# bnbowman/pbccs

Measured on AMD Instinct MI355X. Metric: CCS ZMWs/sec (and GCUPS) at 1/2/4/8 MI355X vs host-CPU ccs, higher is better.
Workload: dtype f64

## Files before the change

pbccs_amd/csrc/arrow_kernels.hip:

```cpp
#include "arrow_device.hpp"
#include "arrow_kernels.hpp"
#include "arrow_score_device.hpp"
#include "coop_chain.hpp"

#include <climits>

namespace pbccs {

__device__ __forceinline__ LaneBand scratch_band(const FillScratch& F, int g, int l, int which)
{
    const long long gm = 2LL * g + which;
    LaneBand m;
    m.range = F.range + gm * F.capCols * 64 + l;
    m.off = F.off + gm * F.capCols * 64 + l;
    m.ls = F.ls + gm * F.capCols * 64 + l;
    m.val = F.val + gm * F.capSlots * 64 + l;
    m.cap = F.capSlots;
    return m;
}

__global__ void __launch_bounds__(64) k_fill(DevBatch B, FillScratch F, const int* __restrict__ reads, int n)
{
    const int t = blockIdx.x * blockDim.x + threadIdx.x;
    if (t >= n) return;
    const int g = t >> 6, l = t & 63;
    const long long tStart = F.trace ? (long long)wall_clock64() : 0;
    const int r = reads[t];
    const int z = B.rZmw[r];
    const int I = B.rLen[r];
    const TplView tv = window_view(B, r);
    const int J = tv.Length();
    if (I < 1 || J < 1 || J + 2 > F.capCols) {
        B.rStatus[r] = (I < 1 || J < 1) ? kFillBadInput : kFillOverflow;
        return;
    }
    const char* rd = B.seqPool + B.rSeqOff[r];
    const Params P = params_for(B, z);
    const LaneBand a = scratch_band(F, g, l, 0);
// ... 140 lines not shown
                if (ok[q] && c < ncol[q]) {
                    const long long bits = __double_as_longlong(tile[ln][q]);
                    (which ? B.bRange : B.aRange)[cb[q] + c] = make_int2((int)(bits & 0xffffffff), (int)(bits >> 32));
                }
            }
            __syncthreads();
            for (int q = w; q < 64; q += 4) {
                const int c = c0 + q;
                tile[q][ln] = __longlong_as_double((c < maxC) ? (long long)F.off[gm + (long long)c * 64 + ln] : 0LL);
            }
            __syncthreads();
            for (int q = w; q < 64; q += 4) {
                const int c = c0 + ln;
                if (ok[q] && c < ncol[q]) (which ? B.bOff : B.aOff)[cb[q] + c] = (int)__double_as_longlong(tile[ln][q]);
            }
            __syncthreads();
        }
        const double* pre = F.pre + (long long)g * (F.capCols + 1) * 64;
        for (int q = w; q < 64; q += 4) {
            const int c = c0 + q;
            tile[q][ln] = (c < maxC + 1) ? pre[(long long)c * 64 + ln] : 0.0;
        }
        __syncthreads();
        for (int q = w; q < 64; q += 4) {
            const int c = c0 + ln;
            if (ok[q] && c < ncol[q] + 1) B.aPre[cb[q] + c] = tile[ln][q];
        }
        __syncthreads();
    }
}

constexpr int kSuffixTile = 2048;

__device__ __forceinline__ double add8(double s, const double* __restrict__ t)
{
    double v[8];
#pragma unroll
    for (int i = 0; i < 8; ++i) v[i] = t[i];
#pragma unroll
    for (int i = 0; i < 8; ++i) s = s + v[i];
    return s;
}

__device__ __forceinline__ void k_suffix_body(DevBatch B, const int* __restrict__ reads, int n, int withPrefix)
{
    __shared__ double tile[kSuffixTile];
    const int r = reads[blockIdx.x];
    if (B.rStatus[r] != kFillOk && B.rStatus[r] != kFillMismatch) return;
    const long long cb = B.rColBase[r];
    const int J = window_view(B, r).Length();
    const double* ls = B.bLs + cb;
    double* suf = B.bSuf + cb;
    const int ncol = J + 1;
    const int lane = threadIdx.x & 63;
    const int wbase = threadIdx.x & ~63;
    for (int k0 = 0; k0 <= ncol; k0 += blockDim.x) {
        const int kb = k0 + wbase;
        const int k = kb + lane;
        double s = 0.0;
        for (int c0 = k0; c0 < ncol; c0 += kSuffixTile) {
            __syncthreads();
            for (int q = threadIdx.x; q < kSuffixTile && c0 + q < ncol; q += blockDim.x) tile[q] = ls[c0 + q];
            __syncthreads();
            const int hi = min(ncol - c0, kSuffixTile);
            int q = max(kb - c0, 0);
            const int headEnd = min(hi, kb + 64 - c0);
            for (; q < headEnd; ++q) {
                const double v = tile[q];
                if (c0 + q >= k) s = s + v;
            }
            for (; q + 8 <= hi; q += 8) s = add8(s, tile + q);
            for (; q < hi; ++q) s = s + tile[q];
        }
        if (k <= ncol) suf[k] = s;
    }
    if (!withPrefix) return;
    if (threadIdx.x != 0) return;
    const double* als = B.aLs + cb;
    double* pre = B.aPre + cb;
    double run = 0.0;
    pre[0] = 0.0;
    int k = 0;
    for (; k + 8 <= ncol; k += 8) {
        double v[8];
#pragma unroll
        for (int q = 0; q < 8; ++q) v[q] = als[k + q];
#pragma unroll
        for (int q = 0; q < 8; ++q) {
            run = run + v[q];
            pre[k + q + 1] = run;
        }
    }
    for (; k < ncol; ++k) {
        run = run + als[k];
        pre[k + 1] = run;
    }
}
__global__ void __launch_bounds__(256) k_suffix(DevBatch B, const int* __restrict__ reads, int n, int withPrefix)
{
    const long long wt0 = wave_t0(B.stats);
    k_suffix_body(B, reads, n, withPrefix);
    wave_ticks(B.stats, kWaveSuffix, wt0);
}

__global__ void __launch_bounds__(256) k_enumerate(DevBatch B, const int* __restrict__ zmws,
                                                   const long long* __restrict__ mutBase,
                                                   const long long* __restrict__ posBase, int* __restrict__ codes,
                                                   int* __restrict__ posOff)
{
    __shared__ int waveSums[4];
    __shared__ int carry;
    const int z = zmws[blockIdx.x];
    const char* T = B.tplPool + B.zFwdOff[z];
    const int L = B.zLen[z];
    int* out = codes + mutBase[blockIdx.x];
    int* po = posOff + posBase[blockIdx.x];
    if (threadIdx.x == 0) carry = 0;
    __syncthreads();
    const int lane = threadIdx.x & 63, wid = threadIdx.x >> 6;
    for (int p0 = 0; p0 < L; p0 += 256) {
        const int p = p0 + threadIdx.x;
        int cnt = 0;
        char cur = 0, prev = '-';
        if (p < L) {
            cur = T[p];
            prev = p > 0 ? T[p - 1] : '-';
            cnt = (p == 0) ? 8 : 6 + (cur != prev ? 1 : 0);
        }
        int incl = cnt;
        for (int d = 1; d < 64; d <<= 1) {
            const int y = __shfl_up(incl, d, 64);
            if (lane >= d) incl += y;
        }
        if (lane == 63) waveSums[wid] = incl;
// ... 943 lines not shown
    int tagSub = -1, tagIns = -1;
    for (int m = po[p]; m < po[p + 1]; ++m) {
        const double s = sc[m];
        const int c = code[m];
        const int type = mut_type(c);
        const double e = s < 0.0 ? exp(s) : 0.0;
        part[0] += type == kIns ? e : 0.0;
        part[1] += type == kDel ? e : 0.0;
        part[2] += type == kSub ? e : 0.0;
        if (type == kSub && (tagSub < 0 || s > bestSub)) { bestSub = s; tagSub = mut_base(c); }
        if (type == kIns && (tagIns < 0 || s > bestIns)) { bestIns = s; tagIns = mut_base(c); }
    }
    const long long o = qvBase[k] + p;
    qv[o] = sum_to_qv(sum);
    R.ins[o] = sum_to_qv(part[0]);
    R.del[o] = sum_to_qv(part[1]);
    R.sub[o] = sum_to_qv(part[2]);
    R.subTag[o] = tagSub < 0 ? 'N' : base_char(tagSub);
    R.insTag[o] = tagIns < 0 ? 'N' : base_char(tagIns);
}

void launch_fill(const DevBatch& B, const FillScratch& F, const int* reads, int n, hipStream_t s)
{
    if (n <= 0) return;
    hipLaunchKernelGGL(k_fill, dim3((n + 63) / 64), dim3(64), 0, s, B, F, reads, n);
}

void launch_compact(const DevBatch& B, const FillScratch& F, const int* reads, int n, hipStream_t s)
{
    if (n <= 0) return;
    hipLaunchKernelGGL(k_compact, dim3((n + 63) / 64), dim3(256), 0, s, B, F, reads, n);
}

void launch_suffix(const DevBatch& B, const int* reads, int n, hipStream_t s, bool withPrefix)
{
    if (n <= 0) return;
    hipLaunchKernelGGL(k_suffix, dim3(n), dim3(256), 0, s, B, reads, n, withPrefix ? 1 : 0);
}

void launch_enumerate(const DevBatch& B, const int* zmws, int n, const long long* mutBase, const long long* posBase,
                      int* codes, int* posOff, hipStream_t s)
{
    if (n <= 0) return;
    hipLaunchKernelGGL(k_enumerate, dim3(n), dim3(256), 0, s, B, zmws, mutBase, posBase, codes, posOff);
}

void launch_score(const DevBatch& B, const ScoreWork& W, long long nWaves, const ScoreScratch& scratch, hipStream_t s,
                  const CkptWork* ck)
{
    if (nWaves <= 0) return;
    const long long blocks = (nWaves + kScoreWaves - 1) / kScoreWaves;
    hipLaunchKernelGGL(k_score, dim3((unsigned)blocks), dim3(64 * kScoreWaves), 0, s, B, W, scratch);
    if (ck && ck->nTasks > 0 && ck->nSlots > 0)
        hipLaunchKernelGGL(k_score_ckpt, dim3((unsigned)ck->nSlots), dim3(64), 0, s, B, W, *ck);
    if (W.edgeCap > 0)
        hipLaunchKernelGGL(k_score_edge, dim3((W.edgeCap + 63) / 64), dim3(64), 0, s, B, W, scratch);
}

void launch_reduce(const DevBatch& B, const ScoreWork& W, long long nMut, double fastThr, double* score,
                   unsigned char* fav, hipStream_t s)
{
    if (nMut <= 0) return;
    hipLaunchKernelGGL(k_reduce, dim3((unsigned)((nMut + 255) / 256)), dim3(256), 0, s, B, W, fastThr, score, fav);
}

void launch_alive(const DevBatch& B, const ScoreWork& W, long long nMut, double fastThr, int readHi,
                  unsigned char* alive, hipStream_t s)
{
    if (nMut <= 0) return;
    hipLaunchKernelGGL(k_alive, dim3((unsigned)((nMut + 255) / 256)), dim3(256), 0, s, B, W, fastThr, readHi, alive);
// ... 35 lines not shown
```

pbccs_amd/csrc/arrow_kernels.hpp:

```cpp
#pragma once

#include <hip/hip_runtime.h>

#include "arrow_device.hpp"

namespace pbccs {

struct ScoreWork {
    int nWork = 0;
    const int* zmw = nullptr;
    const int* nMut = nullptr;
    const long long* mutBase = nullptr;
    const long long* deltaBase = nullptr;
    const long long* waveStart = nullptr;
    const long long* mutStart = nullptr;
    const long long* posStart = nullptr;
    const int* codes = nullptr;
    double* delta = nullptr;
    int* edgeList = nullptr;
    int* edgeCount = nullptr;
    int edgeCap = 0;
    int readLo = 0;
    int readHi = 1 << 30;
    const long long* sel = nullptr;
// ... 59 lines not shown
    int* maxH = nullptr;
    int hcap = 0;
    int readWords = 0;
    int tplWords = 0;
    size_t groupBytes = 0;
    bool prio = false;
    bool chainExit = true;
    bool scan = false;
    double devScale = 1.0;
    int rows = 1;
    double thrMargin = 0x1p-50;
    int regrowSlackDiv = 16;
    unsigned long long* valBump = nullptr;
    long long valLimit = 0;
    long long* rValA = nullptr;
    long long* rValB = nullptr;
    long long* rValCap = nullptr;
    double* colScratch = nullptr;
    int gRows = 0;
    long long* trace = nullptr;
    unsigned long long* work = nullptr;
};
enum FillWork : int {
    kFillWorkCells = 0, kFillWorkTallAbort, kFillWorkRegrow, kFillWorkOverflow, kFillWorkSteps, kFillWorkIssues,
    kFillWorkReads, kFillWorkPasses, kFillWorkSlots
};
size_t coop_group_bytes(int hcap, int readWords, int tplWords);
constexpr int kNarrowGroupLanes = 16;
constexpr int kTallRowsPerLane = 2;
void launch_fill_coop(int G, const DevBatch& B, const CoopFill& F, const int* reads, int n, hipStream_t s);

void launch_fill(const DevBatch& B, const FillScratch& F, const int* reads, int n, hipStream_t s);
void launch_compact(const DevBatch& B, const FillScratch& F, const int* reads, int n, hipStream_t s);
void launch_suffix(const DevBatch& B, const int* reads, int n, hipStream_t s, bool withPrefix = false);
void launch_enumerate(const DevBatch& B, const int* zmws, int n, const long long* mutBase, const long long* posBase,
                      int* codes, int* posOff, hipStream_t s);
void launch_score(const DevBatch& B, const ScoreWork& W, long long nWaves, const ScoreScratch& scratch, hipStream_t s,
                  const CkptWork* ck = nullptr);
void launch_alive(const DevBatch& B, const ScoreWork& W, long long nMut, double fastThr, int readHi,
                  unsigned char* alive, hipStream_t s);
void launch_sel_ranges(const ScoreWork& W, const long long* sel, const long long* count, long long* selBase,
                       int* nSel, hipStream_t s);
void launch_score_wide(const DevBatch& B, const WideTask* tasks, int n, double* delta, hipStream_t s);
void launch_score_wide_refill(const DevBatch& B, const WideTask* tasks, int n, double* delta,
                              const ScoreScratch& scratch, int rowsCap, hipStream_t s);
void launch_reduce(const DevBatch& B, const ScoreWork& W, long long nMut, double fastThr, double* score,
                   unsigned char* fav, hipStream_t s);
void launch_best_subset(int nWork, const long long* selBase, const int* nSel, const int* code, const double* score,
                        int sep, int ldsCap, int* rank, hipStream_t s);
void launch_qv(const DevBatch& B, const ScoreWork& W, long long nPos, const long long* posBase, const int* posOff,
               const double* score, const long long* qvBase, int* qv, hipStream_t s);
struct RichQvOut {
    int* sub = nullptr;
    int* ins = nullptr;
    int* del = nullptr;
    char* subTag = nullptr;
    char* insTag = nullptr;
};
void launch_qv_rich(const DevBatch& B, const ScoreWork& W, long long nPos, const long long* posBase, const int* posOff,
                    const double* score, const long long* qvBase, int* qv, const RichQvOut& R, hipStream_t s);

}
```

pbccs_amd/csrc/engine.hip:

```cpp
#include "engine.hpp"
#include "diploid_kernels.hpp"
#include "refine_repeats.hpp"
#include "strand_kernels.hpp"

#include <hipcub/hipcub.hpp>

#include <algorithm>
#include <mutex>
#include <climits>
#include <cmath>
#include <cstdio>
#include <cstdlib>
#include <cstring>
#include <numeric>
#include <set>
#include <stdexcept>
#include <chrono>
#include <unordered_set>

namespace pbccs {

#define PBCCS_HIP(x)                                                         \
    do {                                                                     \
        hipError_t e_ = (x);                                                 \
        if (e_ != hipSuccess) throw DeviceError(hipGetErrorString(e_));      \
    } while (0)

const char* const kKernelNames[kKernelKinds] = {"k_fill",       "k_suffix",      "k_enumerate", "k_score",
                                                 "k_reduce",     "k_qv",          "k_best_subset", "k_compact",
                                                 "k_fill_tall",  "k_qfill_grp",   "k_qfill_coop", "k_qfill",
                                                 "k_qscore_mid", "k_qscore_multi", "k_score_wide", "k_qv_rich",
                                                 "k_strand_sums", "k_strand_sites"};

namespace {

constexpr int kFillBandHeight = 28;
constexpr double kFillScratchBudget = 24.0 * (1ull << 30);
constexpr int kCoopNarrowRows = 64;
constexpr int kCoopTallRows = 1024;
constexpr size_t kCoopLdsBytes = 60 * 1024;
constexpr int kHybridRows = 1536;
constexpr size_t kHeadroomMargin = 24ull << 30;
constexpr long long kTallFirstDiv = 25;
constexpr int kCkptDefaultK = 8;
constexpr int kCkptDefaultMinLen = 4000;
constexpr int kCkptSlotsMax = 2048;
constexpr long long kCkptSlotBytes = 1ll << 30;
int env_int(const char* name, int dflt)
{
    const char* e = std::getenv(name);
    return e ? std::atoi(e) : dflt;
}
constexpr long long kPhasedMinTasks = 1 << 21;
constexpr size_t kInitialScratch = 1 << 20;
constexpr int kMaxCopySegs = 8;

template <class T>
void upload(DevVec<T>& d, const std::vector<T>& h, hipStream_t s)
{
    d.reserve(std::max<size_t>(h.size(), 1), false);
    if (!h.empty()) PBCCS_HIP(hipMemcpyAsync(d.ptr, h.data(), h.size() * sizeof(T), hipMemcpyHostToDevice, s));
}

void d2h(void* dst, const void* src, size_t bytes, hipStream_t s)
{
    static const bool drain = env_int("PBCCS_D2H_DRAIN", 1) != 0;
    if (!bytes) return;
    if (drain) PBCCS_HIP(hipStreamSynchronize(s));
    PBCCS_HIP(hipMemcpyAsync(dst, src, bytes, hipMemcpyDeviceToHost, s));
}

template <class T>
void download(std::vector<T>& h, const DevVec<T>& d, size_t n, hipStream_t s)
{
    h.resize(n);
    d2h(h.data(), d.ptr, n * sizeof(T), s);
}

struct CopySeg {
    const unsigned int* src;
    unsigned int* dst;
    unsigned long long words;
};
struct CopySegs {
// ... 835 lines not shown
    b.prThird = kMismatchProbability / 3.0;
    b.sdn = zmws_.empty() ? std::exp(12.5) : std::exp(zmws_[0].opt.scoreDiff);
    b.stats = profiling_ ? dStats_.ptr : nullptr;
    return b;
}

void ArrowBatch::FillReads(const std::vector<int>& readsIn)
{
    const StreamScope bound(stream_);
    constexpr int kPaths = 4;
    for (int r : readsIn) EnsureCapacity(r);
    auto promote = [&](int r, int p) {
        HRead& h = reads_[r];
        int q = p + 1;
        if (q == 2 && (long long)h.seq.size() + 1 > 4LL * kCoopTallRows) q = 3;
        h.fillPath = q;
        if (q >= 2 && q < kPaths) {
            const long long I = (long long)h.seq.size(), J = h.te - h.ts;
            const bool ck = ckptAll_ > 0 || (ckptK_ > 0 && J >= ckptMinLen_);
            const long long K = ck ? std::max(ckptAll_, ckptK_) : 1;
            const long long want = (I + 1) * (J + 1) / kTallFirstDiv / K + (ck ? 2 * (kCkptTail + 1) * (I + 1) : 0) + 64;
            if (want > h.valCap) {
                h.valCap = want;
                h.valA = valTop_;
                h.valB = valTop_ + h.valCap;
                valTop_ += 2 * h.valCap;
                descDirty_ = true;
            }
        }
        return q;
    };
    Relayout(readsIn);
    const int firstPath = std::min(std::max(env_int("PBCCS_FILL_FIRST_PATH", 1), 1), 3);
    std::vector<int> todo[kPaths], serial, done;
    for (int r : readsIn) {
        if (reads_[r].fillPath < firstPath) reads_[r].fillPath = firstPath;
        const int p = reads_[r].fillPath;
        if (p >= kPaths) serial.push_back(r);
        else todo[p].push_back(r);
    }
    auto words = [&](int r) {
        return (int)(reads_[r].seq.size() + 7) / 8 + (reads_[r].te - reads_[r].ts + 8) / 8;
    };
    constexpr int tallG = 64;
    const int tallRows = env_int("PBCCS_TALL_ROWS", kTallRowsPerLane) == 1 ? 1 : 2;
    const long long chunk = (long long)tallG * tallRows;
    const long long tallGroupLds = (long long)kCoopLdsBytes;
    auto full_rows = [&](int maxI) { return ((long long)maxI + chunk) / chunk * chunk; };
    constexpr int narrowG = kNarrowGroupLanes;
    constexpr int narrowRows = 1;
    auto rows_for = [&](int p, int maxI, int w) -> int {
        if (p == 0) return 0;
        if (p == 1)
            return (64 / narrowG) * coop_group_bytes(kCoopNarrowRows, w, 0) <= kCoopLdsBytes
                       ? kCoopNarrowRows : 0;
        const long long room = (tallGroupLds - (long long)coop_group_bytes(0, w, 0)) / 16 / 64 * 64;
        const long long full = full_rows(maxI);
        if (p == 2) {
            const long long want = std::min<long long>(kCoopTallRows, full);
            return room >= want ? (int)want : 0;
        }
        const long long hybLds = (long long)env_int("PBCCS_HYBRID_LDS_KB", (int)(kCoopLdsBytes >> 10)) << 10;
        const long long hybRows = env_int("PBCCS_HYBRID_ROWS", kHybridRows);
        const long long hroom = (std::min<long long>(hybLds, 160 << 10) - (long long)coop_group_bytes(0, w, 0)) / 16 / 64 * 64;
        const long long want = std::min(std::min(full, hroom), hybRows);
        return want >= 64 ? (int)want : 0;
// ... 65 lines not shown
        std::vector<int> list;
        for (auto& v : todo) list.insert(list.end(), v.begin(), v.end());
        upload(dList_, list, stream_);
        const DevBatch B = View();
        size_t off = 0;
        const bool forked = !todo[2].empty() || !todo[3].empty();
        const auto tLaunch = std::chrono::steady_clock::now();
        const bool grow = ws_->val.allowVmm;
        long long headroom = 0;
        if (grow) {
            long long want = 1ll << 24;
            for (int p = 2; p < kPaths; ++p)
                for (int r : todo[p]) {
                    const long long I = (long long)reads_[r].seq.size(), J = reads_[r].te - reads_[r].ts;
                    const long long K = std::max(1, reads_[r].ckpt);
                    want += 2 * std::max<long long>(0, (I + 1) * (J + 1) / 7 / K - reads_[r].valCap);
                }
            size_t freeB = 0, totalB = 0;
            PBCCS_HIP(hipMemGetInfo(&freeB, &totalB));
            static const long long margin = (long long)env_int("PBCCS_HEADROOM_MARGIN_GB", (int)(kHeadroomMargin >> 30)) << 30;
            const long long spare = std::max<long long>(0, (long long)freeB - margin);
            headroom = std::min<long long>(want, spare / 4 / (long long)sizeof(double));
            dVal_.reserve((size_t)std::max<long long>(valTop_, 1), true);
            dVal_.try_reserve((size_t)std::max<long long>(valTop_ + headroom, 1));
            dBump_.reserve(1, false);
            const unsigned long long top = (unsigned long long)valTop_;
            PBCCS_HIP(hipMemcpyAsync(dBump_.ptr, &top, sizeof(top), hipMemcpyHostToDevice, stream_));
        }
        const long long valLimit = grow ? (long long)dVal_.cap : 0;
        if (forked) {
            PBCCS_HIP(hipEventRecord(evFork_, stream_));
            PBCCS_HIP(hipStreamWaitEvent(stream2_, evFork_, 0));
        }
        for (int p = 0; p < kPaths; ++p) {
            const int n = (int)todo[p].size();
            if (n == 0) continue;
            int maxI = 1, maxJ = 1;
            for (int r : todo[p]) {
                maxI = std::max(maxI, (int)reads_[r].seq.size());
                maxJ = std::max(maxJ, reads_[r].te - reads_[r].ts);
            }
            CoopFill F;
            F.usedA = dUsedA_.ptr;
            F.usedB = dUsedB_.ptr;
            F.maxH = dMaxH_.ptr;
            F.readWords = (maxI + 7) / 8;
            F.tplWords = (maxJ + 8) / 8;
            F.hcap = rows_for(p, maxI, F.readWords + F.tplWords);
            const int G = p == 1 ? narrowG : tallG;
            F.rows = p == 1 ? narrowRows : tallRows;
            F.prio = p >= 2;
            if (const char* e = std::getenv("PBCCS_FILL_THR_MARGIN"))
                F.thrMargin = std::max(0x1p-50, std::atof(e));
            F.groupBytes = coop_group_bytes(F.hcap, F.readWords, F.tplWords);
            const int full = (int)full_rows(maxI);
            if (p == 3 && full > F.hcap) {
                F.gRows = full - F.hcap;
                dColScratch_.reserve((size_t)n * 2 * F.gRows, false);
                F.colScratch = dColScratch_.ptr;
            }
            if (grow) {
                F.valBump = dBump_.ptr;
                F.valLimit = valLimit;
                F.rValA = pRValA_;
                F.rValB = pRValB_;
                F.rValCap = pRValCap_;
            }
            const int* lp = dList_.ptr + off;
            const hipStream_t st = p <= 1 ? stream_ : stream2_;
            if (fillWork) {
                if (!dFillWork_.ptr) {
                    dFillWork_.reserve(16, false);
                    PBCCS_HIP(hipMemsetAsync(dFillWork_.ptr, 0, 16 * sizeof(unsigned long long), stream_));
                }
                F.work = dFillWork_.ptr;
            }
            if (pathTrace2) {
                dCoopTrace_[p].reserve((size_t)6 * n, false);
                PBCCS_HIP(hipMemsetAsync(dCoopTrace_[p].ptr, 0, sizeof(long long) * 6 * n, st));
                F.trace = dCoopTrace_[p].ptr;
            }
            const int nScan2 = nScan[p];
            if (nScan2 > 0) {
                CoopFill FS = F;
                FS.scan = true;
                if (const char* e = std::getenv("PBCCS_SCAN_DEV_SCALE")) FS.devScale = std::max(1.0, std::atof(e));
                Timed(p == 1 ? kKFill : kKFillTall, [&] { launch_fill_coop(G, B, FS, lp, nScan2, st); }, st);
                PBCCS_HIP(hipGetLastError());
                counters_.fillLaunches += 1;
                counters_.scanReads += nScan2;
                if (n > nScan2) {
                    Timed(p == 1 ? kKFill : kKFillTall, [&] { launch_fill_coop(G, B, F, lp + nScan2, n - nScan2, st); },
                          st);
                    PBCCS_HIP(hipGetLastError());
                    counters_.fillLaunches += 1;
                }
            } else {
                Timed(p == 1 ? kKFill : kKFillTall, [&] { launch_fill_coop(G, B, F, lp, n, st); }, st);
                PBCCS_HIP(hipGetLastError());
                counters_.fillLaunches += 1;
            }
            off += n;
        }
        if (forked) {
            PBCCS_HIP(hipEventRecord(evJoin_, stream2_));
            PBCCS_HIP(hipStreamWaitEvent(stream_, evJoin_, 0));
            static const bool joinSync = std::getenv("PBCCS_DBG_JOINSYNC") && std::getenv("PBCCS_DBG_JOINSYNC")[0] == '1';
            if (joinSync) PBCCS_HIP(hipStreamSynchronize(stream2_));
        }
        std::vector<int> st, fl, ua, ub, mh;
        std::vector<double> bl, dv;
        unsigned long long bump = (unsigned long long)valTop_;
        {
            std::vector<Xfer> xs{xfer_dl(mh, dMaxH_, R), xfer_dl(st, dRStatus_, R), xfer_dl(fl, dRFlips_, R),
                                 xfer_dl(bl, dRBaseline_, R), xfer_dl(ua, dUsedA_, R), xfer_dl(ub, dUsedB_, R)};
            if (anyScan) xs.push_back(xfer_dl(dv, dRDev_, R));
            if (grow) xs.push_back(Xfer{dBump_.ptr, &bump, sizeof(bump)});
            download_packed(xs, ws_->xStage, hXStage_, stream_);
        }
        if (grow && bump != (unsigned long long)valTop_) {
            std::vector<long long> va, vb, vc;
            va.resize(R);
            vb.resize(R);
            vc.resize(R);
            d2h(va.data(), pRValA_, R * sizeof(long long), stream_);
            d2h(vb.data(), pRValB_, R * sizeof(long long), stream_);
            d2h(vc.data(), pRValCap_, R * sizeof(long long), stream_);
            PBCCS_HIP(hipStreamSynchronize(stream_));
            for (auto& v : todo)
                for (int r : v) {
                    reads_[r].valA = va[r];
                    reads_[r].valB = vb[r];
// ... 47 lines not shown
                    else next[q].push_back(r);
                    continue;
                }
                if (st[r] == kFillUncertain) {
                    h.exact = true;
                    counters_.uncertainReads += 1;
                    for (int bit = 0; bit < 4; ++bit) counters_.uncertainWhy[bit] += (fl[r] >> bit) & 1;
                    next[p].push_back(r);
                    continue;
                }
                if (st[r] == kFillOverflow) {
                    const long long need = std::max(ua[r], ub[r]);
                    h.valCap = std::max(need + need / 16 + 64, h.valCap + 1);
                    h.valA = valTop_;
                    h.valB = valTop_ + h.valCap;
                    valTop_ += 2 * h.valCap;
                    descDirty_ = true;
                    next[p].push_back(r);
                    continue;
                }
                h.status = st[r];
                h.flips = fl[r];
                h.baseline = bl[r];
                h.dev = !dv.empty() ? dv[r] : 0.0;
                h.filled = true;
                h.usedA = ua[r];
                h.usedB = ub[r];
                if (p >= 1) h.maxH = mh[r];
                if (st[r] == kFillOk || st[r] == kFillMismatch) done.push_back(r);
            }
        }
        for (int p = 0; p < kPaths; ++p) todo[p].swap(next[p]);
    }
    if (!done.empty()) {
        upload(dList_, done, stream_);
        const DevBatch B = View();
        Timed(kKSuffix, [&] { launch_suffix(B, dList_.ptr, (int)done.size(), stream_, true); });
        PBCCS_HIP(hipGetLastError());
        PBCCS_HIP(hipStreamSynchronize(stream_));
    }
    if (!serial.empty()) FillReadsSerial(serial);
    (void)counters();
}

void ArrowBatch::FillReadsSerial(const std::vector<int>& readsIn)
{
    const StreamScope bound(stream_);
    std::vector<int> todo(readsIn);
    for (int r : todo)
        if (reads_[r].ckpt != 0) {
            reads_[r].ckpt = 0;
            descDirty_ = true;
        }
    for (int r : todo) EnsureCapacity(r);
    int H = kFillBandHeight;
    for (int attempt = 0; !todo.empty(); ++attempt) {
        if (attempt > 8) throw DeviceError("band storage keeps overflowing");
        std::stable_sort(todo.begin(), todo.end(), [&](int x, int y) {
            return reads_[x].te - reads_[x].ts > reads_[y].te - reads_[y].ts;
        });
        UploadDescriptors();
        const size_t R = reads_.size();
        dUsedA_.reserve(std::max<size_t>(R, 1), true);
        dUsedB_.reserve(std::max<size_t>(R, 1), true);
        std::vector<int> again;
        size_t pos = 0;
        while (pos < todo.size()) {
            const int capCols = reads_[todo[pos]].te - reads_[todo[pos]].ts + 2;
            const long long capSlots = (long long)capCols * H + 64;
            const double perGroup = 2.0 * capSlots * 64 * 8 + 2.0 * capCols * 64 * 20 + (capCols + 1.0) * 64 * 8;
// ... 29 lines not shown
            std::vector<int> st, fl, ua, ub;
            std::vector<double> bl;
            download_packed({xfer_dl(st, dRStatus_, R), xfer_dl(fl, dRFlips_, R), xfer_dl(bl, dRBaseline_, R),
                             xfer_dl(ua, dUsedA_, R), xfer_dl(ub, dUsedB_, R)},
                            ws_->xStage, hXStage_, stream_);
            if (trace) TraceSummary(n, H, capSlots);
            for (int r : chunk) {
                HRead& h = reads_[r];
                if (st[r] == kFillOverflow) {
                    again.push_back(r);
                    continue;
                }
                h.status = st[r];
                h.flips = fl[r];
                h.baseline = bl[r];
                h.dev = 0.0;
                h.filled = true;
                h.usedA = ua[r];
                h.usedB = ub[r];
                if (st[r] == kFillOk || st[r] == kFillMismatch) {
                    const long long need = std::max(ua[r], ub[r]);
                    if (need > h.valCap) {
                        h.valCap = need + need / 4 + 64;
                        h.valA = valTop_;
                        h.valB = valTop_ + h.valCap;
                        valTop_ += 2 * h.valCap;
                        descDirty_ = true;
                    }
                }
            }
            UploadDescriptors();
            const DevBatch B2 = View();
            Timed(kKCompact, [&] { launch_compact(B2, F, dList_.ptr, (int)n, stream_); });
            Timed(kKSuffix, [&] { launch_suffix(B2, dList_.ptr, (int)n, stream_); });
            PBCCS_HIP(hipGetLastError());
            PBCCS_HIP(hipStreamSynchronize(stream_));
            pos += n;
        }
        todo.swap(again);
        H *= 2;
    }
}

void ArrowBatch::TraceSummary(size_t n, int H, long long capSlots)
{
    std::vector<long long> tr;
    download(tr, dTrace_, 8 * n, stream_);
    PBCCS_HIP(hipStreamSynchronize(stream_));
    long long t0 = LLONG_MAX, t1 = 0, maxDur = 0, maxCells = 0, sumCells = 0, sumPass = 0, maxPass = 0;
    double sumDur = 0;
    long long done = 0;
    for (size_t t = 0; t < n; ++t) {
        const long long* e = &tr[8 * t];
        if (e[1] <= 0) continue;
        ++done;
        t0 = std::min(t0, e[0]);
        t1 = std::max(t1, e[1]);
        maxDur = std::max(maxDur, e[1] - e[0]);
        sumDur += double(e[1] - e[0]);
        maxCells = std::max(maxCells, e[2]);
        sumCells += e[2];
        sumPass += e[3];
        maxPass = std::max(maxPass, e[3]);
    }
    std::fprintf(stderr,
                 "[fill-trace] lanes=%zu done=%lld H=%d capSlots=%lld span_ms=%.3f maxlane_ms=%.3f avglane_ms=%.3f "
                 "cells avg=%.0f max=%lld passes avg=%.2f max=%lld\n",
// ... 1231 lines not shown
```

pbccs_amd/csrc/fill_coop.hip:

```cpp
#include "arrow_device.hpp"
#include "arrow_kernels.hpp"
#include "coop_chain.hpp"

#include <algorithm>
#include <cstdlib>
#include <stdexcept>

namespace pbccs {
namespace {

using namespace coop;

template <int G>
struct Task {
    Group<G> g;
    int I, J, L, start;
    const unsigned* rdW;
    const unsigned* tpW;
    const double* ctx;
    double* lds0;
    double* lds1;
    double* glob0;
    double* glob1;
    int hcap;
    int rowsCap;
    bool gcol;
    int ckK;
    bool chainExit;
    int slackDiv;
    double prNot, prThird, sdn;
    double sdnInvLow;
    double sdnInvHigh;
    double devScale;
    double sdnInv;
    int r;
    double* pool;
    unsigned long long* bump;
    long long limit;
    long long* gA;
    long long* gB;
    long long* gCap;

    __device__ __forceinline__ int uni(int x) const
    {
        if constexpr (G == 64) return __builtin_amdgcn_readfirstlane(x);
        return x;
    }

    template <int R>
    __device__ __forceinline__ int lrow(int k) const
    {
        static_assert(R <= 2, "the split layout has two planes");
        return R > 1 ? (k & 1) * (hcap >> 1) + (k >> 1) : k;
    }
    template <int R>
    __device__ __forceinline__ double* cptr(int b, int k) const
    {
        if (!gcol) return lds0 + (b ? hcap : 0) + lrow<R>(k);
        return k < hcap ? lds0 + (b ? hcap : 0) + lrow<R>(k) : glob0 + (b ? glob1 - glob0 : 0) + (k - hcap);
    }
    template <int R>
    __device__ __forceinline__ double cget(int b, int k) const { return *cptr<R>(b, k); }
    template <int R>
    __device__ __forceinline__ void cset(int b, int k, double v) const { *cptr<R>(b, k) = v; }
    template <int R>
    __device__ __forceinline__ double* lptr(int b, int c, int r) const
    {
        static_assert(R <= 2, "the split layout has two planes");
        return lds0 + (b ? hcap : 0) + (R > 1 ? r * (hcap >> 1) : 0) + c * G + g.lane;
    }
    template <int R>
    __device__ __forceinline__ double lget_sel(int b, int s, int h) const
    {
        static_assert(R <= 2, "the split layout has two planes");
// ... 122 lines not shown
    double* no = mIsAlpha ? nb : na;
    copy_vals<G>(T.g.lane, no, o.val, keepO);
    m.val = nm;
    o.val = no;
    m.cap = cap;
    o.cap = cap;
    if (T.g.lane == 0) {
        T.gA[T.r] = (long long)base;
        T.gB[T.r] = (long long)base + cap;
        T.gCap[T.r] = cap;
    }
    return true;
}

template <int G>
__device__ double finish_log_scales(const Task<G>& T, const Band& m, int J)
{
    __builtin_amdgcn_fence(__ATOMIC_ACQ_REL, "workgroup");
    double s = 0.0;
    if (T.g.lane == 0) {
        int k = 0;
        for (; k + 7 <= J; k += 8) {
            double v[8];
#pragma unroll
            for (int q = 0; q < 8; ++q) v[q] = m.L(k + q);
#pragma unroll
            for (int q = 0; q < 8; ++q) s = s + v[q];
        }
        for (; k <= J; ++k) s = s + m.L(k);
    }
    return T.g.bcast(s, 0);
}

#ifndef PBCCS_TALL_PREFETCH
#define PBCCS_TALL_PREFETCH 1
#endif
template <int G, int R, bool SCAN, bool GC>
__device__ PassOut coop_alpha(const Task<G>& T, Band& a, Band& o, bool guided, bool selfValid, bool& ovf, long long keepO,
                              Work& W)
{
    constexpr int CH = G * R;
    constexpr bool PF = GC || (G == 64 && PBCCS_TALL_PREFETCH && !SCAN);
    constexpr bool PFS = GC || (G == 64 && PBCCS_TALL_PREFETCH);
    const Band* guide = guided ? &o : nullptr;
    const int I = T.I, J = T.J, lane = T.g.lane;
    PassOut out{0, 0, 0.0, 0.0, false, !selfValid, false, 1, 0.0, 0};
    bool counting = false;
    (void)keepO;
    if (a.cap < 1) ovf = true;
    if (lane == 0) {
        if (!ovf) a.V(0) = 1.0;
        a.R(0) = make_int2(0, 1);
        a.O(0) = 0;
        a.L(0) = 0.0;
    }
    int prev = 0, cur = 1;
    if (lane == 0) T.template cset<R>(prev, 0, 1.0);
    int pb = 0, pe = 1;
    double D = 0.0;
    int unc = 0;
    long long used = 1, stored = 1;
    int hb = 1, he = 1;
    int prevCtx = kCtxZero;
    int curBase = T.TBase(0), curCtx = T.TCtx(0);
    int tA = T.TBase(1), tB = T.TBase(2);
    double myF = 1.0;
// ... 293 lines not shown
        col_fence(T.gcol && nc * CH > T.hcap);
        prev ^= 1;
        cur ^= 1;
        pb = b;
        pe = e;
        prevCtx = curCtx;
        curBase = nextBase;
        curCtx = nextCtx;
        tA = tB;
        tB = tC;
        he = e;
        hb = nhb;
    }
    const double em = (T.RB(I - 1) == T.TBase(J - 1)) ? T.prNot : T.prThird;
    const bool lastIn = I - 1 >= pb && I - 1 < pe;
    const double lik = (lastIn ? T.template cget<R>(prev, I - 1 - pb) : 0.0) * em;
    const double c = (0.0 < lik) ? lik : 0.0;
    double v = lik, ls = 0.0;
    if (c != 0.0 && c != 1.0) { v = lik / c; ls = log(c); }
    if (!ovf && !counting && stored + 1 > a.cap) {
        if (T.bump) counting = true;
        else ovf = true;
    }
    out.regrow = counting;
    if (lane == 0 && !counting) {
        if (!ovf) a.V(stored) = v;
        a.R(J) = make_int2(I, I + 1);
        a.O(J) = (int)stored;
        a.L(J) = ls;
    }
    out.used = used + 1;
    out.stored = stored + 1;
    out.last = v;
    if (!counting) out.sumL = finish_log_scales<G>(T, a, J);
    if constexpr (SCAN) {
        out.dev = T.devScale * (1.01 * (D + 4.0 * kUnitRoundoff) +
                                2.0 * (double)(J + 4) * kUnitRoundoff * (fabs(out.sumL) + fabs(log(fmax(v, 1e-300))) + 64.0));
        out.unc = unc | ((lastIn && v == 0.0) ? 1 : 0);
    }
    return out;
}

template <int G, int R, bool SCAN, bool GC>
__device__ PassOut coop_beta(const Task<G>& T, Band& bm, Band& o, bool guided, bool selfValid, bool& ovf, long long keepO,
                             Work& W)
{
    constexpr int CH = G * R;
    constexpr bool PF = GC || (G == 64 && PBCCS_TALL_PREFETCH && !SCAN);
    constexpr bool PFS = GC || (G == 64 && PBCCS_TALL_PREFETCH);
    const Band* guide = guided ? &o : nullptr;
    const int I = T.I, J = T.J, lane = T.g.lane;
    PassOut out{0, 0, 0.0, 0.0, false, !selfValid, false, 1, 0.0, 0};
    bool counting = false;
    (void)keepO;
    if (bm.cap < 1) ovf = true;
    if (lane == 0) {
        if (!ovf) bm.V(0) = 1.0;
        bm.R(J) = make_int2(I, I + 1);
        bm.O(J) = 0;
        bm.L(J) = 0.0;
    }
    int nxt = 0, cur = 1;
    if (lane == 0) T.template cset<R>(nxt, 0, 1.0);
    int pb = I, pe = I + 1;
    double D = 0.0;
    int unc = 0;
    long long used = 1, stored = 1;
// ... 396 lines not shown
    T.g.lane = lane;
    T.g.base = (int)threadIdx.x & ~(G - 1);
    T.I = T.uni(I);
    T.J = T.uni(J);
    T.L = tv.L;
    T.start = tv.start;
    T.rdW = rdW;
    T.tpW = tpW;
    T.ctx = ctx;
    T.lds0 = col;
    T.lds1 = col + F.hcap;
    T.glob0 = GC ? F.colScratch + (size_t)t * 2 * F.gRows : nullptr;
    T.glob1 = GC ? T.glob0 + F.gRows : nullptr;
    T.hcap = F.hcap;
    T.rowsCap = GC ? F.hcap + F.gRows : F.hcap;
    T.gcol = GC;
    T.chainExit = F.chainExit;
    T.ckK = B.rCkpt ? B.rCkpt[r] : 0;
    T.slackDiv = max(1, F.regrowSlackDiv);
    T.prNot = B.prNot;
    T.prThird = B.prThird;
    T.sdn = B.sdn;
    T.sdnInvLow = (1.0 / B.sdn) * (1.0 - F.thrMargin);
    T.sdnInvHigh = (1.0 / B.sdn) * (1.0 + F.thrMargin);
    T.devScale = F.devScale;
    T.sdnInv = 1.0 / B.sdn;
    T.r = r;
    T.pool = B.valPool;
    T.bump = F.valBump;
    T.limit = F.valLimit;
    T.gA = F.rValA;
    T.gB = F.rValB;
    T.gCap = F.rValCap;

    const long long cb = B.rColBase[r];
    Band a, bm;
    a.range = B.aRange + cb;
    a.off = B.aOff + cb;
    a.ls = B.aLs + cb;
    a.val = B.valPool + B.rValA[r];
    a.cap = B.rValCap[r];
    bm.range = B.bRange + cb;
    bm.off = B.bOff + cb;
    bm.ls = B.bLs + cb;
    bm.val = B.valPool + B.rValB[r];
    bm.cap = B.rValCap[r];

    bool ovf = false;
    long long needA = 0, needB = 0;
    unsigned long long cells = 0, passes = 0;
    int flips = 0;
    Work W{F.work != nullptr, 0, 0};
    unsigned long long regrowCells = 0, abortCells = 0;
    bool tallAbort = false;
    PassOut pa{0, 0, 0.0, 0.0, false, false, false, 0, 0.0, 0}, pb{0, 0, 0.0, 0.0, false, false, false, 0, 0.0, 0};
    int maxH = 0;
    long long ua = 0, ub = 0;
    long long sa = 0, sb = 0;
    const int maxSize = (int)(0.5 + kRebandFrac * (I + 1) * (J + 1));
    bool mismatched = false;
    int uncAny = 0;
    int unchanged = 0;
    int regrows = 0;
    for (int step = 0;; ++step) {
        bool doAlpha;
        if (step < 2) doAlpha = step == 0;
// ... 181 lines not shown
```

Baseline: 3593.

## Restructure suffix kernel, fuse prefix into alpha fill, overlap suffix with fills

Rewrites the suffix-sum kernel so each lane computes several start columns (templated rows, default 4), which reuses each loaded log-scale value across more outputs. An optional scalar-load variant is selectable by environment variable. The alpha prefix sum is now written inside the fill's final log-scale reduction instead of the separate suffix pass. The suffix launch is moved to run per fill slice on the same stream rather than once after all paths join. The trade-offs are more register pressure and extra serial stores by lane 0 during the fill finish.

Result: no change. 3617, median of 6 (+0.7%).

```diff
diff --git a/pbccs_amd/csrc/arrow_kernels.hip b/pbccs_amd/csrc/arrow_kernels.hip
--- a/pbccs_amd/csrc/arrow_kernels.hip
+++ b/pbccs_amd/csrc/arrow_kernels.hip
@@ -4,6 +4,7 @@
 #include "coop_chain.hpp"
 
 #include <climits>
+#include <stdexcept>
 
 namespace pbccs {
 
@@ -210,6 +211,99 @@
 
 constexpr int kSuffixTile = 2048;
 
+typedef double suffix_d8 __attribute__((ext_vector_type(8)));
+template <bool SC>
+__device__ __forceinline__ double suffix_ld1(const double* __restrict__ t)
+{
+    if constexpr (SC) {
+        double v;
+        asm volatile("s_load_dwordx2 %0, %1, 0x0\n\ts_waitcnt lgkmcnt(0)" : "=&s"(v) : "s"(t) : "memory");
+        return v;
+    } else {
+        return *t;
+    }
+}
+
+template <int R, bool SC>
+__device__ __forceinline__ void add8r(double (&s)[R], const double* __restrict__ t)
+{
+    double v[8];
+    if constexpr (SC) {
+        suffix_d8 x;
+        asm volatile("s_load_dwordx16 %0, %1, 0x0\n\ts_waitcnt lgkmcnt(0)" : "=&s"(x) : "s"(t) : "memory");
+#pragma unroll
+        for (int i = 0; i < 8; ++i) v[i] = x[i];
+    } else {
+#pragma unroll
+        for (int i = 0; i < 8; ++i) v[i] = t[i];
+    }
+#pragma unroll
+    for (int i = 0; i < 8; ++i)
+#pragma unroll
+        for (int a = 0; a < R; ++a) s[a] = s[a] + v[i];
+}
+
+template <int R, bool SC>
+__device__ __forceinline__ void k_suffix_rows(const DevBatch& B, const int* __restrict__ reads)
+{
+    __shared__ double tile[SC ? 1 : kSuffixTile];
+    const int r = reads[blockIdx.x];
+    if (B.rStatus[r] != kFillOk && B.rStatus[r] != kFillMismatch) return;
+    const long long cb = B.rColBase[r];
+    const int J = window_view(B, r).Length();
+    const double* __restrict__ ls = B.bLs + cb;
+    double* __restrict__ suf = B.bSuf + cb;
+    const int ncol = J + 1;
+    const int lane = threadIdx.x & 63;
+    const int wbase = __builtin_amdgcn_readfirstlane((int)(threadIdx.x >> 6)) * 64 * R;
+    for (int k0 = 0; k0 <= ncol; k0 += 256 * R) {
+        const int kb = k0 + wbase;
+        double s[R];
+#pragma unroll
+        for (int a = 0; a < R; ++a) s[a] = 0.0;
+        for (int c0 = k0; c0 < ncol; c0 += SC ? ncol : kSuffixTile) {
+            const double* __restrict__ t = tile;
+            if constexpr (SC) {
+                t = ls + c0;
+            } else {
+                __syncthreads();
+                for (int q = threadIdx.x; q < kSuffixTile && c0 + q < ncol; q += blockDim.x) tile[q] = ls[c0 + q];
+                __syncthreads();
+            }
+            const int hi = SC ? ncol - c0 : min(ncol - c0, kSuffixTile);
+            int q = max(kb - c0, 0);
+#pragma unroll
+            for (int m = 0; m < R; ++m) {
+                const int end = min(hi, kb + 64 * (m + 1) - c0);
+                for (; q < end; ++q) {
+                    const double v = suffix_ld1<SC>(t + q);
+#pragma unroll
+                    for (int a = 0; a < m; ++a) s[a] = s[a] + v;
+                    if (c0 + q >= kb + 64 * m + lane) s[m] = s[m] + v;
+                }
+            }
+            for (; q + 8 <= hi; q += 8) add8r<R, SC>(s, t + q);
+            for (; q < hi; ++q) {
+                const double v = suffix_ld1<SC>(t + q);
+#pragma unroll
+                for (int a = 0; a < R; ++a) s[a] = s[a] + v;
+            }
+        }
+#pragma unroll
+        for (int a = 0; a < R; ++a) {
+            const int k = kb + 64 * a + lane;
+            if (k <= ncol) suf[k] = s[a];
+        }
+    }
+}
+template <int R, bool SC>
+__global__ void __launch_bounds__(256) k_suffix(DevBatch B, const int* __restrict__ reads)
+{
+    const long long wt0 = wave_t0(B.stats);
+    k_suffix_rows<R, SC>(B, reads);
+    wave_ticks(B.stats, kWaveSuffix, wt0);
+}
+
 __device__ __forceinline__ double add8(double s, const double* __restrict__ t)
 {
     double v[8];
@@ -220,7 +314,7 @@
     return s;
 }
 
-__device__ __forceinline__ void k_suffix_body(DevBatch B, const int* __restrict__ reads, int n, int withPrefix)
+__device__ __forceinline__ void k_suffix_ref_body(DevBatch B, const int* __restrict__ reads, int n, int withPrefix)
 {
     __shared__ double tile[kSuffixTile];
     const int r = reads[blockIdx.x];
@@ -274,10 +368,10 @@
         pre[k + 1] = run;
     }
 }
-__global__ void __launch_bounds__(256) k_suffix(DevBatch B, const int* __restrict__ reads, int n, int withPrefix)
+__global__ void __launch_bounds__(256) k_suffix_ref(DevBatch B, const int* __restrict__ reads, int n, int withPrefix)
 {
     const long long wt0 = wave_t0(B.stats);
-    k_suffix_body(B, reads, n, withPrefix);
+    k_suffix_ref_body(B, reads, n, withPrefix);
     wave_ticks(B.stats, kWaveSuffix, wt0);
 }
 
@@ -1287,10 +1381,22 @@
     hipLaunchKernelGGL(k_compact, dim3((n + 63) / 64), dim3(256), 0, s, B, F, reads, n);
 }
 
-void launch_suffix(const DevBatch& B, const int* reads, int n, hipStream_t s, bool withPrefix)
+void launch_suffix(const DevBatch& B, const int* reads, int n, hipStream_t s, const SuffixMode& m)
 {
     if (n <= 0) return;
-    hipLaunchKernelGGL(k_suffix, dim3(n), dim3(256), 0, s, B, reads, n, withPrefix ? 1 : 0);
+    if (m.ref) {
+        hipLaunchKernelGGL(k_suffix_ref, dim3(n), dim3(256), 0, s, B, reads, n, m.refPrefix ? 1 : 0);
+        return;
+    }
+    using K = void (*)(DevBatch, const int*);
+    K k = nullptr;
+    switch (m.rows) {
+    case 2: k = m.scalar ? (K)k_suffix<2, true> : (K)k_suffix<2, false>; break;
+    case 4: k = m.scalar ? (K)k_suffix<4, true> : (K)k_suffix<4, false>; break;
+    case 8: k = m.scalar ? (K)k_suffix<8, true> : (K)k_suffix<8, false>; break;
+    default: throw std::runtime_error("k_suffix is built for 2, 4 and 8 start columns per lane");
+    }
+    hipLaunchKernelGGL(k, dim3(n), dim3(256), 0, s, B, reads);
 }
 
 void launch_enumerate(const DevBatch& B, const int* zmws, int n, const long long* mutBase, const long long* posBase,
diff --git a/pbccs_amd/csrc/arrow_kernels.hpp b/pbccs_amd/csrc/arrow_kernels.hpp
--- a/pbccs_amd/csrc/arrow_kernels.hpp
+++ b/pbccs_amd/csrc/arrow_kernels.hpp
@@ -115,7 +115,14 @@
 
 void launch_fill(const DevBatch& B, const FillScratch& F, const int* reads, int n, hipStream_t s);
 void launch_compact(const DevBatch& B, const FillScratch& F, const int* reads, int n, hipStream_t s);
-void launch_suffix(const DevBatch& B, const int* reads, int n, hipStream_t s, bool withPrefix = false);
+constexpr int kSuffixRows = 4;
+struct SuffixMode {
+    int rows = kSuffixRows;
+    bool scalar = false;
+    bool ref = false;
+    bool refPrefix = false;
+};
+void launch_suffix(const DevBatch& B, const int* reads, int n, hipStream_t s, const SuffixMode& m = SuffixMode{});
 void launch_enumerate(const DevBatch& B, const int* zmws, int n, const long long* mutBase, const long long* posBase,
                       int* codes, int* posOff, hipStream_t s);
 void launch_score(const DevBatch& B, const ScoreWork& W, long long nWaves, const ScoreScratch& scratch, hipStream_t s,
diff --git a/pbccs_amd/csrc/engine.hip b/pbccs_amd/csrc/engine.hip
--- a/pbccs_amd/csrc/engine.hip
+++ b/pbccs_amd/csrc/engine.hip
@@ -50,6 +50,16 @@
 {
     const char* e = std::getenv(name);
     return e ? std::atoi(e) : dflt;
+}
+SuffixMode suffix_mode(bool prefix)
+{
+    SuffixMode m;
+    m.ref = env_int("PBCCS_SUFFIX_REF", 0) == 1;
+    m.refPrefix = prefix;
+    const int rows = env_int("PBCCS_SUFFIX_ROWS", kSuffixRows);
+    m.rows = rows == 2 || rows == 8 ? rows : kSuffixRows;
+    m.scalar = env_int("PBCCS_SUFFIX_SCALAR", 0) == 1;
+    return m;
 }
 constexpr long long kPhasedMinTasks = 1 << 21;
 constexpr size_t kInitialScratch = 1 << 20;
@@ -951,6 +961,8 @@
     };
     Relayout(readsIn);
     const int firstPath = std::min(std::max(env_int("PBCCS_FILL_FIRST_PATH", 1), 1), 3);
+    const SuffixMode sfx = suffix_mode(true);
+    const bool sfxAfterJoin = env_int("PBCCS_SUFFIX_AFTER_JOIN", 0) == 1;
     std::vector<int> todo[kPaths], serial, done;
     for (int r : readsIn) {
         if (reads_[r].fillPath < firstPath) reads_[r].fillPath = firstPath;
@@ -1082,6 +1094,11 @@
             PBCCS_HIP(hipEventRecord(evFork_, stream_));
             PBCCS_HIP(hipStreamWaitEvent(stream2_, evFork_, 0));
         }
+        auto sums = [&](const int* slice, int n, hipStream_t st) {
+            if (sfxAfterJoin) return;
+            Timed(kKSuffix, [&] { launch_suffix(B, slice, n, st, sfx); }, st);
+            PBCCS_HIP(hipGetLastError());
+        };
         for (int p = 0; p < kPaths; ++p) {
             const int n = (int)todo[p].size();
             if (n == 0) continue;
@@ -1137,17 +1154,20 @@
                 if (const char* e = std::getenv("PBCCS_SCAN_DEV_SCALE")) FS.devScale = std::max(1.0, std::atof(e));
                 Timed(p == 1 ? kKFill : kKFillTall, [&] { launch_fill_coop(G, B, FS, lp, nScan2, st); }, st);
                 PBCCS_HIP(hipGetLastError());
+                sums(lp, nScan2, st);
                 counters_.fillLaunches += 1;
                 counters_.scanReads += nScan2;
                 if (n > nScan2) {
                     Timed(p == 1 ? kKFill : kKFillTall, [&] { launch_fill_coop(G, B, F, lp + nScan2, n - nScan2, st); },
                           st);
                     PBCCS_HIP(hipGetLastError());
+                    sums(lp + nScan2, n - nScan2, st);
                     counters_.fillLaunches += 1;
                 }
             } else {
                 Timed(p == 1 ? kKFill : kKFillTall, [&] { launch_fill_coop(G, B, F, lp, n, st); }, st);
                 PBCCS_HIP(hipGetLastError());
+                sums(lp, n, st);
                 counters_.fillLaunches += 1;
             }
             off += n;
@@ -1261,10 +1281,10 @@
         }
         for (int p = 0; p < kPaths; ++p) todo[p].swap(next[p]);
     }
-    if (!done.empty()) {
+    if (sfxAfterJoin && !done.empty()) {
         upload(dList_, done, stream_);
         const DevBatch B = View();
-        Timed(kKSuffix, [&] { launch_suffix(B, dList_.ptr, (int)done.size(), stream_, true); });
+        Timed(kKSuffix, [&] { launch_suffix(B, dList_.ptr, (int)done.size(), stream_, sfx); });
         PBCCS_HIP(hipGetLastError());
         PBCCS_HIP(hipStreamSynchronize(stream_));
     }
@@ -1360,7 +1380,7 @@
             UploadDescriptors();
             const DevBatch B2 = View();
             Timed(kKCompact, [&] { launch_compact(B2, F, dList_.ptr, (int)n, stream_); });
-            Timed(kKSuffix, [&] { launch_suffix(B2, dList_.ptr, (int)n, stream_); });
+            Timed(kKSuffix, [&] { launch_suffix(B2, dList_.ptr, (int)n, stream_, suffix_mode(false)); });
             PBCCS_HIP(hipGetLastError());
             PBCCS_HIP(hipStreamSynchronize(stream_));
             pos += n;
diff --git a/pbccs_amd/csrc/fill_coop.hip b/pbccs_amd/csrc/fill_coop.hip
--- a/pbccs_amd/csrc/fill_coop.hip
+++ b/pbccs_amd/csrc/fill_coop.hip
@@ -40,6 +40,7 @@
     long long* gA;
     long long* gB;
     long long* gCap;
+    long long preOff;
 
     __device__ __forceinline__ int uni(int x) const
     {
@@ -228,6 +229,33 @@
     return T.g.bcast(s, 0);
 }
 
+template <int G>
+__device__ double finish_log_scales_pre(const Task<G>& T, const Band& m, int J)
+{
+    __builtin_amdgcn_fence(__ATOMIC_ACQ_REL, "workgroup");
+    double s = 0.0;
+    if (T.g.lane == 0) {
+        double* pre = m.ls + T.preOff;
+        pre[0] = 0.0;
+        int k = 0;
+        for (; k + 7 <= J; k += 8) {
+            double v[8];
+#pragma unroll
+            for (int q = 0; q < 8; ++q) v[q] = m.L(k + q);
+#pragma unroll
+            for (int q = 0; q < 8; ++q) {
+                s = s + v[q];
+                pre[k + q + 1] = s;
+            }
+        }
+        for (; k <= J; ++k) {
+            s = s + m.L(k);
+            pre[k + 1] = s;
+        }
+    }
+    return T.g.bcast(s, 0);
+}
+
 #ifndef PBCCS_TALL_PREFETCH
 #define PBCCS_TALL_PREFETCH 1
 #endif
@@ -587,7 +615,7 @@
     out.used = used + 1;
     out.stored = stored + 1;
     out.last = v;
-    if (!counting) out.sumL = finish_log_scales<G>(T, a, J);
+    if (!counting) out.sumL = finish_log_scales_pre<G>(T, a, J);
     if constexpr (SCAN) {
         out.dev = T.devScale * (1.01 * (D + 4.0 * kUnitRoundoff) +
                                 2.0 * (double)(J + 4) * kUnitRoundoff * (fabs(out.sumL) + fabs(log(fmax(v, 1e-300))) + 64.0));
@@ -1050,6 +1078,7 @@
     T.gA = F.rValA;
     T.gB = F.rValB;
     T.gCap = F.rValCap;
+    T.preOff = B.aPre - B.aLs;
 
     const long long cb = B.rColBase[r];
     Band a, bm;
```
